# nyashiki/nshogi-engine

Hardware: NVIDIA B200
Metric: nn_leaf_evals_per_sec_batch256 (higher is better)
Workload: dtype bf16

## Files before the change

### nshogi-engine_b200/binding.py

```python
from __future__ import annotations

import ctypes as C
import os
from typing import Optional

import numpy as np

HERE = os.path.dirname(os.path.abspath(__file__))
LIB_PATH = os.path.join(HERE, "libnsb.so")

NUM_SQUARES = 81
POLICY_SIZE = 2187
FEATURE_CHANNELS = 86
MAX_LEGAL_MOVES = 593
CACHE_MAX_MOVES = 164
DECODE_PROBS = 0
DECODE_LOGITS = 1
DECODE_BOTH = 2
DECODE_NAN_FALLBACK = 0x100
ROW_SKIP_SOFTMAX = 1

FEATURE_BITBOARD = np.dtype([("lo", "<u8"), ("hi", "<u8")])
POSITION = np.dtype(
    {
# ... 255 lines not shown


class Event:

    def __init__(self):
        p = _P()
        _check(lib().nsb_event_create(C.byref(p)), "nsb_event_create")
        self._p = p

    def record(self, ctx: "Context", slot: int = 0):
        _check(ctx._l.nsb_event_record(self._p, ctx._h, slot), "nsb_event_record")

    def sync(self):
        _check(lib().nsb_event_sync(self._p), "nsb_event_sync")

    def elapsed_ms(self, stop: "Event") -> float:
        ms = C.c_float(0)
        _check(lib().nsb_event_elapsed_ms(self._p, stop._p, C.byref(ms)), "nsb_event_elapsed_ms")
        return float(ms.value)

    def destroy(self):
        if self._p is not None:
            lib().nsb_event_destroy(self._p)
            self._p = None


class Context:

    def __init__(self, desc: NetDesc, batch_max: int, slots: int = 1, gpu: int = 0,
                 blob: Optional[np.ndarray] = None, seed: Optional[int] = None, diag: bool = False):
        self.desc = desc
        self.batch_max = batch_max
        self.slots = slots
        self._l = diag_lib() if diag else lib()
        h = _P()
        _check(self._l.nsb_create(C.byref(h), gpu, batch_max, slots, C.byref(desc)), "nsb_create")
        self._h = h
        if blob is None and seed is not None:
            blob = random_blob(desc, seed)
        if blob is not None:
            self.load_weights(blob)

    def close(self):
        if self._h is not None:
            self._l.nsb_destroy(self._h)
            self._h = None

    def __enter__(self):
        return self

    def __exit__(self, *a):
        self.close()

    def load_weights(self, blob: np.ndarray):
        blob = np.ascontiguousarray(blob, dtype=np.float32)
        _check(self._l.nsb_load_weights(self._h, blob.ctypes.data, blob.size), "nsb_load_weights")

    def bind_thread(self):
        _check(self._l.nsb_bind_thread(self._h), "nsb_bind_thread")

    def eval_async(self, slot, features, n, policy, win, draw):
        _check(self._l.nsb_eval_async(self._h, slot, _ptr(features), n, _ptr(policy), _ptr(win), _ptr(draw)),
               "nsb_eval_async")

    def eval_decode_async(self, slot, features, n, move_off, move_idx, mode, legal_out, win, draw, nan_flag=None):
        _check(self._l.nsb_eval_decode_async(self._h, slot, _ptr(features), n, _ptr(move_off), _ptr(move_idx), mode,
                                           _ptr(legal_out), _ptr(win), _ptr(draw), _ptr(nan_flag)),
               "nsb_eval_decode_async")

    def eval_positions_async(self, slot, positions, n, policy, win, draw):
        _check(self._l.nsb_eval_positions_async(self._h, slot, _ptr(positions), n, _ptr(policy), _ptr(win),
                                              _ptr(draw)), "nsb_eval_positions_async")

    def eval_positions_decode_async(self, slot, positions, n, move_off, move_idx, mode, legal_out, win, draw,
                                    nan_flag=None):
        _check(self._l.nsb_eval_positions_decode_async(self._h, slot, _ptr(positions), n, _ptr(move_off),
                                                     _ptr(move_idx), mode, _ptr(legal_out), _ptr(win), _ptr(draw),
                                                     _ptr(nan_flag)), "nsb_eval_positions_decode_async")

    def await_(self, slot=0):
        _check(self._l.nsb_await(self._h, slot), "nsb_await")

    def is_computing(self, slot=0) -> bool:
        rc = self._l.nsb_is_computing(self._h, slot)
        if rc < 0:
            _check(rc, "nsb_is_computing")
        return rc == 1

    def eval_device(self, slot, d_features, n, d_policy, d_win, d_draw):
        _check(self._l.nsb_eval_device(self._h, slot, _ptr(d_features), n, _ptr(d_policy), _ptr(d_win), _ptr(d_draw)),
               "nsb_eval_device")

    def eval_decode_device(self, slot, d_features, n, d_off, d_idx, mode, d_policy, d_legal, d_win, d_draw, d_flag):
        _check(self._l.nsb_eval_decode_device(self._h, slot, _ptr(d_features), n, _ptr(d_off), _ptr(d_idx), mode,
                                            _ptr(d_policy), _ptr(d_legal), _ptr(d_win), _ptr(d_draw), _ptr(d_flag)),
               "nsb_eval_decode_device")

    def extract_device(self, slot, d_features, n, channels, channels_first, d_planes):
        _check(self._l.nsb_extract_device(self._h, slot, _ptr(d_features), n, channels, int(channels_first),
                                        _ptr(d_planes)), "nsb_extract_device")

    def pack_positions_device(self, slot, d_positions, n, d_features):
        _check(self._l.nsb_pack_positions_device(self._h, slot, _ptr(d_positions), n, _ptr(d_features)),
               "nsb_pack_positions_device")

    def decode_device(self, slot, d_policy, d_win, d_draw, n, d_off, d_idx, mode, d_legal, d_flag):
        _check(self._l.nsb_decode_device(self._h, slot, _ptr(d_policy), _ptr(d_win), _ptr(d_draw), n, _ptr(d_off),
                                       _ptr(d_idx), mode, _ptr(d_legal), _ptr(d_flag)), "nsb_decode_device")

    def decode_device_ex(self, slot, d_policy, d_win, d_draw, n, d_off, d_idx, mode, d_row_flags, d_legal, d_logits, d_flag):
        _check(self._l.nsb_decode_device_ex(self._h, slot, _ptr(d_policy), _ptr(d_win), _ptr(d_draw), n, _ptr(d_off),
                                          _ptr(d_idx), mode, _ptr(d_row_flags), _ptr(d_legal), _ptr(d_logits), _ptr(d_flag)),
               "nsb_decode_device_ex")

    def cache_create(self, memory_mb: int):
        _check(self._l.nsb_cache_create(self._h, memory_mb), "nsb_cache_create")

    def cache_clear(self):
        _check(self._l.nsb_cache_clear(self._h), "nsb_cache_clear")

    def cache_num_bundles(self) -> int:
        return int(self._l.nsb_cache_num_bundles(self._h))

    def cache_store_device(self, slot, d_hashes, n, d_off, d_legal, d_win, d_draw, d_skip=None, d_stored=None):
        _check(self._l.nsb_cache_store_device(self._h, slot, _ptr(d_hashes), n, _ptr(d_off), _ptr(d_legal), _ptr(d_win),
                                            _ptr(d_draw), _ptr(d_skip), _ptr(d_stored)), "nsb_cache_store_device")

    def cache_probe_device(self, slot, d_hashes, n, d_off, d_legal, d_win, d_draw, d_hit, d_miss_idx, d_miss_count):
        _check(self._l.nsb_cache_probe_device(self._h, slot, _ptr(d_hashes), n, _ptr(d_off), _ptr(d_legal), _ptr(d_win),
                                            _ptr(d_draw), _ptr(d_hit), _ptr(d_miss_idx), _ptr(d_miss_count)),
               "nsb_cache_probe_device")

    def eval_cached_decode_async(self, slot, features, n, hashes, move_off, move_idx, mode, legal_out, win, draw,
                                 nan_flag=None, hit_flag=None):
        _check(self._l.nsb_eval_cached_decode_async(self._h, slot, _ptr(features), n, _ptr(hashes), _ptr(move_off),
                                                  _ptr(move_idx), mode, _ptr(legal_out), _ptr(win), _ptr(draw),
                                                  _ptr(nan_flag), _ptr(hit_flag)), "nsb_eval_cached_decode_async")

    def eval_positions_cached_decode_async(self, slot, positions, n, hashes, move_off, move_idx, mode, legal_out, win,
                                           draw, nan_flag=None, hit_flag=None):
        _check(self._l.nsb_eval_positions_cached_decode_async(self._h, slot, _ptr(positions), n, _ptr(hashes),
                                                            _ptr(move_off), _ptr(move_idx), mode, _ptr(legal_out),
                                                            _ptr(win), _ptr(draw), _ptr(nan_flag), _ptr(hit_flag)),
               "nsb_eval_positions_cached_decode_async")

    def eval_cached_decode_device(self, slot, d_features, n, d_hashes, d_off, d_idx, mode, d_legal, d_win, d_draw,
                                  d_flag, d_hit):
        _check(self._l.nsb_eval_cached_decode_device(self._h, slot, _ptr(d_features), n, _ptr(d_hashes), _ptr(d_off),
                                                   _ptr(d_idx), mode, _ptr(d_legal), _ptr(d_win), _ptr(d_draw),
                                                   _ptr(d_flag), _ptr(d_hit)), "nsb_eval_cached_decode_device")

    def debug_trunk_timeline(self, slot, d_features, n, positions=False):
        nl = 2 * self.desc.blocks + 2
        out = np.zeros(nl * 4 + 16 + 3 * 1024, dtype=np.uint64)
        fn = self._l.nsb_debug_trunk_timeline_positions if positions else self._l.nsb_debug_trunk_timeline
        _check(fn(self._h, slot, _ptr(d_features), n, out.ctypes.data, out.size), "nsb_debug_trunk_timeline")
        return out[:nl * 4].reshape(nl, 4), out[nl * 4:]

    def eval_request_async(self, slot, n, move_off, move_idx, mode, legal_out, win, draw, features=None, positions=None,
                           hashes=None, order_out=None, nan_flag=None, hit_flag=None, row_flags=None, logits_out=None):
        r = DecodeRequest(_ptr(features), _ptr(positions), n, _ptr(hashes), _ptr(move_off), _ptr(move_idx), mode,
                          _ptr(legal_out), _ptr(order_out), _ptr(win), _ptr(draw), _ptr(nan_flag), _ptr(hit_flag),
                          _ptr(row_flags), _ptr(logits_out))
        _check(self._l.nsb_eval_request_async(self._h, slot, C.byref(r)), "nsb_eval_request_async")

    def cache_attach(self, owner: "Context"):
        _check(self._l.nsb_cache_attach(self._h, owner._h), "nsb_cache_attach")

    def set_io_mode(self, direct: bool):
        _check(self._l.nsb_set_io_mode(self._h, 1 if direct else 0), "nsb_set_io_mode")

    def io_mode(self) -> str:
        return "direct" if self._l.nsb_io_mode(self._h) == 1 else "staged"

    def stream(self, slot=0) -> int:
        return self._l.nsb_stream(self._h, slot) or 0

    def set_timing(self, on: bool):
        _check(self._l.nsb_set_timing(self._h, int(on)), "nsb_set_timing")

    def trunk_time(self):
        s, n = C.c_double(0), C.c_uint64(0)
        _check(self._l.nsb_trunk_time(self._h, C.byref(s), C.byref(n)), "nsb_trunk_time")
        return float(s.value), int(n.value)

    def trunk_time_reset(self):
        _check(self._l.nsb_trunk_time_reset(self._h), "nsb_trunk_time_reset")

    def trunk_kernel_name(self) -> str:
        return self._l.nsb_trunk_kernel_name(self._h).decode()

    def launch_count(self) -> int:
        return int(self._l.nsb_launch_count(self._h))
```

### nshogi-engine_b200/csrc/epilogue.cuh

```cuda
#pragma once
#include <stdint.h>

#include "umma.cuh"

namespace nsb {

__host__ __device__ constexpr bool is_real_slot(int n) { return (n % 100) < 90 && ((n % 100) % 10) < 9; }

template <int NCG>
struct EpilogueMask {
    uint32_t m[NCG * 4];
    template <int COL0>
    __device__ __forceinline__ void init_at(int lane) {
#pragma unroll
        for (int G = 0; G < NCG * 4; ++G) {
            uint32_t v = 0;
#pragma unroll
            for (int q4 = 0; q4 < 4; ++q4) {
                const int n = COL0 + 8 * G + 2 * q4;
                const uint32_t c = (is_real_slot(n) ? 0x0000FFFFu : 0u) | (is_real_slot(n + 1) ? 0xFFFF0000u : 0u);
                v = (lane & 3) == q4 ? c : v;
            }
            m[G] = v;
        }
    }
    __device__ __forceinline__ void init(int col0, int lane) {
        if (col0 == 0) init_at<0>(lane);
        else init_at<96>(lane);
    }
};

template <int NCG, bool kResidual, int LBS = 2>
__device__ __forceinline__ void epilogue_half(int lb, uint32_t taddr, uint32_t buf, uint32_t pitch, int chunk0,
                                              int col0, const float (&bias)[4], const EpilogueMask<NCG>& mask,
                                              int lane) {
    const int mk = lane >> 3, mi = lane & 7;
    uint32_t v[NCG][16];
#pragma unroll
    for (int cg = 0; cg < NCG; ++cg) tmem_ld_16x256b_x4(taddr + ((uint32_t)(lb * 16) << 16) + cg * 32, v[cg]);
    const uint32_t row_addr =
        buf + (uint32_t)(chunk0 + lb * LBS + (mk & 1)) * pitch + (uint32_t)(col0 + 8 * (mk >> 1) + mi) * 16u;
    uint32_t xr[NCG][2][4];
    if (kResidual) {
#pragma unroll
        for (int cg = 0; cg < NCG; ++cg)
#pragma unroll
            for (int h = 0; h < 2; ++h)
                ldmatrix_x4_trans(row_addr + (uint32_t)(cg * 32 + h * 16) * 16u, xr[cg][h][0], xr[cg][h][1],
                                  xr[cg][h][2], xr[cg][h][3]);
    }
    tmem_ld_wait();
    const float b0 = lb ? bias[2] : bias[0], b1 = lb ? bias[3] : bias[1];
    const uint64_t bb0 = pack_f32x2(b0, b0), bb1 = pack_f32x2(b1, b1);
#pragma unroll
    for (int cg = 0; cg < NCG; ++cg)
#pragma unroll
        for (int h = 0; h < 2; ++h) {
            uint32_t p[4];
#pragma unroll
            for (int m = 0; m < 4; ++m) {
                const int g = 2 * h + (m >> 1), rh = m & 1;
                uint64_t x = add_f32x2(pack_u32x2(v[cg][4 * g + 2 * rh + 0], v[cg][4 * g + 2 * rh + 1]), rh ? bb1 : bb0);
                if (kResidual) x = add_f32x2(x, pack_u32x2(xr[cg][h][m] << 16, xr[cg][h][m] & 0xFFFF0000u));
                p[m] = pack_relu_bf16x2(x) & mask.m[cg * 4 + g];
            }
            stmatrix_x4_trans(row_addr + (uint32_t)(cg * 32 + h * 16) * 16u, p[0], p[1], p[2], p[3]);
        }
}

template <int NCG, bool kResidual>
__device__ __forceinline__ void epilogue_warp(uint32_t taddr, uint32_t buf, uint32_t pitch, int chunk0, int col0,
                                              const float (&bias)[4], const EpilogueMask<NCG>& mask, int lane) {
#pragma unroll
    for (int lb = 0; lb < 2; ++lb)
        epilogue_half<NCG, kResidual>(lb, taddr, buf, pitch, chunk0, col0, bias, mask, lane);
}

}
```

### nshogi-engine_b200/csrc/nsb_api.cu

```cuda
#include <cuda_runtime.h>
#include <stdarg.h>
#include <stdio.h>
#include <stdlib.h>
#include <string.h>

#include <map>
#include <mutex>
#include <new>
#include <vector>

#include "nsb_internal.h"
#ifdef NSB_DIAG
#include "../../include/nsb_diag.h"
#endif

namespace nsb {

static thread_local char g_err[512] = "";

void set_error(const char* fmt, ...) {
    va_list ap;
    va_start(ap, fmt);
    vsnprintf(g_err, sizeof g_err, fmt, ap);
    va_end(ap);
// ... 863 lines not shown
    r.features = features;
    r.n = n;
    r.hashes = hashes;
    r.move_off = move_off;
    r.move_idx = move_idx;
    r.mode = mode;
    r.legal_out = legal_out;
    r.win = win;
    r.draw = draw;
    r.nan_flag = nan_flag;
    r.hit_flag = hit_flag;
    int rc = check_cache(c, slot, "nsb_eval_cached_decode_async");
    if (rc) return rc;
    if (!features || !hashes) {
        set_error("nsb_eval_cached_decode_async: null buffer or bad mode");
        return NSB_ERR_INVALID;
    }
    return eval_request(c, slot, r, "nsb_eval_cached_decode_async");
}

int nsb_eval_positions_cached_decode_async(nsb_ctx* c, int slot, const nsb_position* positions, size_t n,
                                           const uint64_t* hashes, const uint32_t* move_off, const uint16_t* move_idx,
                                           int mode, float* legal_out, float* win, float* draw, uint8_t* nan_flag,
                                           uint8_t* hit_flag) {
    nsb_decode_request r{};
    r.positions = positions;
    r.n = n;
    r.hashes = hashes;
    r.move_off = move_off;
    r.move_idx = move_idx;
    r.mode = mode;
    r.legal_out = legal_out;
    r.win = win;
    r.draw = draw;
    r.nan_flag = nan_flag;
    r.hit_flag = hit_flag;
    int rc = check_cache(c, slot, "nsb_eval_positions_cached_decode_async");
    if (rc) return rc;
    if (!positions || !hashes) {
        set_error("nsb_eval_positions_cached_decode_async: null buffer or bad mode");
        return NSB_ERR_INVALID;
    }
    return eval_request(c, slot, r, "nsb_eval_positions_cached_decode_async");
}

static int eval_request(nsb_ctx* c, int slot, const nsb_decode_request& r, const char* who) {
    int rc = r.hashes ? check_cache(c, slot, who) : check_ctx(c, slot);
    if (rc) return rc;
    const size_t n = r.n;
    if ((rc = check_batch(c, n, true))) return rc;
    if ((r.features != nullptr) == (r.positions != nullptr) || !r.move_off || !r.move_idx || !r.legal_out || !r.win || !r.draw ||
        !mode_ok(r.mode)) {
        set_error("%s: null buffer or bad mode", who);
        return NSB_ERR_INVALID;
    }
    if (r.positions && (rc = check_positions_net(c, who))) return rc;
    if (n == 0) return 0;
    if ((rc = check_offsets(r.move_off, n, who))) return rc;
    const size_t total = r.move_off[n];
    const bool both = (r.mode & NSB_DECODE_MODE_MASK) == NSB_DECODE_BOTH;
    const uint8_t* row_flags = both ? r.row_flags : nullptr;
    float* logits_out = both ? r.logits_out : nullptr;
    Slot& s = c->slots[slot];
    const size_t in_bytes = r.features ? n * (size_t)c->desc.in_channels * sizeof(nsb_feature_bitboard) : n * sizeof(nsb_position);
    const void* in = r.features ? (const void*)r.features : (const void*)r.positions;

    EvalArgs a{};
    a.n = (int)n;
    a.decode_mode = r.mode;
    const bool direct = c->direct_io && (r.features || c->fuse_pack) && host_mapped(in, in_bytes) &&
                        decode_buffers_mapped(n, total, r.move_off, r.move_idx, r.legal_out, r.win, r.draw, r.nan_flag) &&
                        (!r.hashes || host_mapped(r.hashes, n * sizeof(uint64_t))) && (!r.hit_flag || host_mapped(r.hit_flag, n)) &&
                        (!r.order_out || host_mapped(r.order_out, (total ? total : 1) * sizeof(uint16_t))) &&
                        (!row_flags || host_mapped(row_flags, n)) &&
                        (!logits_out || host_mapped(logits_out, (total ? total : 1) * sizeof(float)));
    const uint64_t* hashes = r.hashes;
    uint8_t* hit = r.hit_flag ? r.hit_flag : s.d_hit;
    if (direct) {
        a.features = r.features;
        a.positions = r.positions;
        a.win = r.win;
        a.draw = r.draw;
        a.move_off = r.move_off;
        a.move_idx = r.move_idx;
        a.legal_out = r.legal_out;
        a.order_out = r.order_out;
        a.nan_flag = r.nan_flag ? r.nan_flag : (r.hashes ? s.d_flag : nullptr);
        a.row_flags = row_flags;
        a.logits_out = logits_out;
    } else {
        NSB_CUDA(cudaMemcpyAsync(r.features ? (void*)s.d_feat : (void*)s.d_pos, in, in_bytes, cudaMemcpyHostToDevice, s.stream));
        a.features = s.d_feat;
        if (r.positions && (rc = stage1(c, s, n, &a.positions))) return rc;
        if (r.hashes) {
            NSB_CUDA(cudaMemcpyAsync(s.d_hash, r.hashes, n * sizeof(uint64_t), cudaMemcpyHostToDevice, s.stream));
            hashes = s.d_hash;
            hit = s.d_hit;
        }
        NSB_CUDA(cudaMemcpyAsync(s.d_off, r.move_off, (n + 1) * sizeof(uint32_t), cudaMemcpyHostToDevice, s.stream));
        if (total)
            NSB_CUDA(cudaMemcpyAsync(s.d_idx, r.move_idx, total * sizeof(uint16_t), cudaMemcpyHostToDevice, s.stream));
        a.win = s.d_win;
        a.draw = s.d_draw;
        a.move_off = s.d_off;
        a.move_idx = s.d_idx;
        a.legal_out = s.d_legal;
        a.order_out = r.order_out ? s.d_order : nullptr;
        a.nan_flag = s.d_flag;
        if (row_flags) {
            NSB_CUDA(cudaMemcpyAsync(s.d_rowflags, row_flags, n, cudaMemcpyHostToDevice, s.stream));
            a.row_flags = s.d_rowflags;
        }
        if (logits_out) {
            if (!s.d_logits) NSB_CUDA(cudaMalloc(&s.d_logits, (size_t)c->batch_max * NSB_MAX_LEGAL_MOVES * sizeof(float)));
            a.logits_out = s.d_logits;
        }
    }
    if (r.hashes) {
        NSB_CUDA(cudaMemsetAsync(s.d_miss_count, 0, sizeof(int), s.stream));
        int k = launch_cache_probe(c->cache, hashes, n, a.move_off, a.legal_out, a.win, a.draw, hit, a.nan_flag, s.d_miss_idx,
                                   s.d_miss_count, s.stream, a.order_out, r.mode, a.row_flags, a.logits_out);
        NSB_CUDA(cudaGetLastError());
        c->launches += (uint64_t)k;
        a.index = s.d_miss_idx;
        a.count = s.d_miss_count;
        a.hashes = hashes;
        a.cache = c->cache;
    }
    if ((rc = run_trunk(c, s, a))) return rc;
    if (direct) return 0;
    if (total) {
        NSB_CUDA(cudaMemcpyAsync(r.legal_out, s.d_legal, total * sizeof(float), cudaMemcpyDeviceToHost, s.stream));
        if (r.order_out)
            NSB_CUDA(cudaMemcpyAsync(r.order_out, s.d_order, total * sizeof(uint16_t), cudaMemcpyDeviceToHost, s.stream));
        if (logits_out)
            NSB_CUDA(cudaMemcpyAsync(logits_out, s.d_logits, total * sizeof(float), cudaMemcpyDeviceToHost, s.stream));
    }
    NSB_CUDA(cudaMemcpyAsync(r.win, s.d_win, n * sizeof(float), cudaMemcpyDeviceToHost, s.stream));
    NSB_CUDA(cudaMemcpyAsync(r.draw, s.d_draw, n * sizeof(float), cudaMemcpyDeviceToHost, s.stream));
    if (r.nan_flag) NSB_CUDA(cudaMemcpyAsync(r.nan_flag, s.d_flag, n, cudaMemcpyDeviceToHost, s.stream));
    if (r.hashes && r.hit_flag) NSB_CUDA(cudaMemcpyAsync(r.hit_flag, s.d_hit, n, cudaMemcpyDeviceToHost, s.stream));
    return 0;
}

#ifdef NSB_DIAG
static int debug_timeline(nsb_ctx* c, int slot, const nsb_feature_bitboard* d_features, const nsb_position* d_positions,
                          size_t n, uint64_t* host_stamps, size_t max_stamps) {
    int rc = check_ctx(c, slot);
    if (rc) return rc;
    if (!c->loaded || (!d_features && !d_positions) || !host_stamps || n == 0) {
        set_error("nsb_debug_trunk_timeline: bad arguments or weights not loaded");
        return NSB_ERR_INVALID;
    }
    const size_t need = (size_t)c->net.num_layers * 4 + 16 + 3 * 1024;
    if (max_stamps < need) {
        set_error("nsb_debug_trunk_timeline: need room for %zu stamps", need);
        return NSB_ERR_INVALID;
    }
    Slot& s = c->slots[slot];
    unsigned long long* d_t = nullptr;
    NSB_CUDA(cudaMalloc(&d_t, need * 8));
    NSB_CUDA(cudaMemsetAsync(d_t, 0, need * 8, s.stream));
    EvalArgs a{};
    a.features = d_features;
    a.positions = d_positions;
    a.n = (int)n;
    a.policy = s.d_policy;
    a.win = s.d_win;
    a.draw = s.d_draw;
    a.timeline = d_t;
    if (n > (size_t)c->batch_max) {
        cudaFree(d_t);
        set_error("nsb_debug_trunk_timeline: n exceeds batch_max");
        return NSB_ERR_INVALID;
    }
    rc = run_trunk(c, s, a);
    if (rc == 0) {
        cudaError_t e = cudaStreamSynchronize(s.stream);
        if (e == cudaSuccess) e = cudaMemcpy(host_stamps, d_t, need * 8, cudaMemcpyDeviceToHost);
        if (e != cudaSuccess) {
            set_error("nsb_debug_trunk_timeline: %s", cudaGetErrorString(e));
            rc = NSB_ERR_CUDA;
        }
    }
    cudaFree(d_t);
    return rc;
}

int nsb_debug_trunk_timeline(nsb_ctx* c, int slot, const nsb_feature_bitboard* d_features, size_t n,
                             uint64_t* host_stamps, size_t max_stamps) {
    return debug_timeline(c, slot, d_features, nullptr, n, host_stamps, max_stamps);
}

int nsb_debug_trunk_timeline_positions(nsb_ctx* c, int slot, const nsb_position* d_positions, size_t n,
                                       uint64_t* host_stamps, size_t max_stamps) {
    return debug_timeline(c, slot, nullptr, d_positions, n, host_stamps, max_stamps);
}

#endif

int nsb_extract_device(nsb_ctx* c, int slot, const nsb_feature_bitboard* d_features, size_t n, int channels,
                       int channels_first, float* d_planes) {
    int rc = check_ctx(c, slot);
    if (rc) return rc;
    if (!d_features || !d_planes || channels < 1 || channels > 1024) {
        set_error("nsb_extract_device: bad arguments");
        return NSB_ERR_INVALID;
    }
    int k = launch_extract(d_features, n, channels, channels_first, d_planes, c->slots[slot].stream);
    if (k < 0) return k;
    NSB_CUDA(cudaGetLastError());
    c->launches += (uint64_t)k;
    return 0;
}

int nsb_pack_positions_device(nsb_ctx* c, int slot, const nsb_position* d_positions, size_t n,
                              nsb_feature_bitboard* d_features) {
    int rc = check_ctx(c, slot);
    if (rc) return rc;
    if (!d_positions || !d_features) {
        set_error("nsb_pack_positions_device: null buffer");
        return NSB_ERR_INVALID;
    }
    int k = launch_pack_positions(d_positions, n, d_features, c->slots[slot].stream);
    if (k < 0) return k;
    NSB_CUDA(cudaGetLastError());
    c->launches += (uint64_t)k;
    return 0;
}

int nsb_decode_device(nsb_ctx* c, int slot, const float* d_policy, const float* d_win, const float* d_draw,
                      size_t n, const uint32_t* d_move_off, const uint16_t* d_move_idx, int mode,
                      float* d_legal_out, uint8_t* d_nan_flag) {
    int rc = check_ctx(c, slot);
    if (rc) return rc;
    return nsb_decode_device_ex(c, slot, d_policy, d_win, d_draw, n, d_move_off, d_move_idx, mode, nullptr, d_legal_out,
                                nullptr, d_nan_flag);
}

int nsb_decode_device_ex(nsb_ctx* c, int slot, const float* d_policy, const float* d_win, const float* d_draw,
                         size_t n, const uint32_t* d_move_off, const uint16_t* d_move_idx, int mode,
                         const uint8_t* d_row_flags, float* d_legal_out, float* d_logits_out, uint8_t* d_nan_flag) {
    int rc = check_ctx(c, slot);
    if (rc) return rc;
    if (!d_policy || !d_win || !d_draw || !d_move_off || !d_move_idx || !d_legal_out || !mode_ok(mode)) {
        set_error("nsb_decode_device: null buffer or bad mode");
        return NSB_ERR_INVALID;
    }
    int k = launch_decode(d_policy, d_win, d_draw, n, d_move_off, d_move_idx, mode, d_legal_out, d_nan_flag,
                          c->slots[slot].stream, d_row_flags, d_logits_out);
    if (k < 0) return k;
    NSB_CUDA(cudaGetLastError());
    c->launches += (uint64_t)k;
    return 0;
}

void* nsb_stream(nsb_ctx* c, int slot) {
    if (check_ctx(c, slot)) return nullptr;
    return c->slots[slot].stream;
}

int nsb_set_timing(nsb_ctx* c, int enabled) {
    if (!c) {
        set_error("null ctx");
        return NSB_ERR_INVALID;
    }
    c->timing = enabled != 0;
    return 0;
}

int nsb_trunk_time(nsb_ctx* c, double* sum_ms, uint64_t* launches) {
    if (!c) {
        set_error("null ctx");
        return NSB_ERR_INVALID;
    }
    if (sum_ms) *sum_ms = c->trunk_ms;
    if (launches) *launches = c->trunk_launches;
    return 0;
}

int nsb_trunk_time_reset(nsb_ctx* c) {
    if (!c) {
        set_error("null ctx");
        return NSB_ERR_INVALID;
    }
    c->trunk_ms = 0.0;
    c->trunk_launches = 0;
    return 0;
}

uint64_t nsb_launch_count(nsb_ctx* c) { return c ? c->launches : 0; }


int nsb_host_alloc(void** out, size_t bytes) {
    if (!out) return NSB_ERR_INVALID;
    NSB_CUDA(cudaHostAlloc(out, bytes ? bytes : 1, cudaHostAllocPortable | cudaHostAllocMapped));
    std::lock_guard<std::mutex> lock(g_host_mu);
    g_host_allocs[(uintptr_t)*out] = HostRange{bytes ? bytes : 1, true, HostKind::Alloc};
    return 0;
}
int nsb_host_alloc_near(void** out, size_t bytes, int gpu) {
    if (!out) return NSB_ERR_INVALID;
    int node = -1;
    void* p = alloc_near_gpu(bytes ? bytes : 1, gpu, &node);
    if (!p) {
        set_error("nsb_host_alloc_near: mmap of %zu bytes failed", bytes);
        return NSB_ERR_NOMEM;
// ... 173 lines not shown
```

### nshogi-engine_b200/csrc/trunk_tmem.cu

```cuda
#include <cuda_bf16.h>
#include <cuda_runtime.h>
#include <stdint.h>

#include "trunk_common.cuh"

namespace nsb {

namespace {

template <int NGRP_>
struct TmemGeom {
    static constexpr int C = 128;
    static constexpr int KCH = C / 8;
    static constexpr int NGRP = NGRP_;
    static constexpr int NPOS = 2;
    static constexpr int QPOS = NGRP * NPOS;
    static constexpr int NCOLS = NPOS * 96;
    static constexpr int GUARD = 12;
    static constexpr int SPITCH = (GUARD + NCOLS + 11) | 1;
    static constexpr int BUF_BYTES = ((KCH * SPITCH * 16 + 127) / 128) * 128;
    static constexpr int KC64 = C / 64;
    static constexpr int TMEM_COLS = 256 * NGRP;
    static constexpr int A_COL0 = NGRP * NCOLS;
    static constexpr int A_STAGES = 4 * NGRP;
    static constexpr int A_STAGE_COLS = 16;
    static constexpr int THREADS = 128 * (2 + NGRP);
    static constexpr int GRP_THREADS = 128;
    static constexpr int EPI_WARPS = GRP_THREADS / 32;
    static constexpr int MMA_WARP = 4 + 4 * NGRP;
    static constexpr int MIN_BLOCKS = NGRP == 1 ? 2 : 1;
    static constexpr int PRODUCER_REGS = 72, EPI_REGS = NGRP == 1 ? 128 : 168, MMA_REGS = 40;
    static constexpr int NBARS = 2 * A_STAGES + 2;
    static constexpr int SCRATCH_BYTES = ((NPOS * kPolicySize * 4 + 15) / 16) * 16;
    static constexpr int FEAT_BYTES = NPOS * kMaxInChannels * 16;
    static constexpr int VBUF_BYTES = ((NPOS * 81 * 4 + 15) / 16) * 16;
    static constexpr int RED_BYTES = ((EPI_WARPS * NPOS * 2 * 4 + NPOS * 2 * 4 + 15) / 16) * 16;
    static constexpr int GRP_BYTES = 2 * BUF_BYTES;
    static constexpr int OFF_BUF_A = 0;
    static constexpr int OFF_BUF_B = BUF_BYTES;
    static constexpr int OFF_VBUF = NGRP * GRP_BYTES;
    static constexpr int OFF_RED = OFF_VBUF + NGRP * VBUF_BYTES;
    static constexpr int OFF_BARS = OFF_RED + NGRP * RED_BYTES;
    static constexpr int SMEM_BYTES = OFF_BARS + NBARS * 8 + 16 + 128;
    static_assert(BUF_BYTES == 55040, "each group has the duo kernel's activation layout");
    static_assert(NGRP > 1 || (OFF_VBUF == 110080 && OFF_RED == 110736 && OFF_BARS == 110816 && SMEM_BYTES == 111040),
                  "one group keeps the duo kernel's shared memory map");
    static_assert(SCRATCH_BYTES <= BUF_BYTES && FEAT_BYTES <= BUF_BYTES, "aliases fit into buffer A");
    static_assert(A_COL0 + A_STAGES * A_STAGE_COLS == TMEM_COLS, "accumulators + the ring fill the allocation");
    static_assert(MIN_BLOCKS * (SMEM_BYTES + 1024) <= 233472, "MIN_BLOCKS CTAs per SM");
    static_assert(128 * (PRODUCER_REGS + NGRP * EPI_REGS + MMA_REGS) <= 65536 / MIN_BLOCKS,
                  "re-balanced registers of MIN_BLOCKS CTAs fit the SM");
};

template <int NGRP>
__device__ __forceinline__ void trunk_tmem_body(const DeviceNet& net, const EvalArgs& a) {
    using G = TmemGeom<NGRP>;
    constexpr int C = G::C;
    extern __shared__ uint8_t smem_raw[];
    uint8_t* smem = reinterpret_cast<uint8_t*>(((uintptr_t)smem_raw + 127) & ~(uintptr_t)127);
    const uint32_t sbase = smem_u32(smem);
    const uint32_t bars = sbase + G::OFF_BARS;
    auto bar_afull = [&](int s) { return bars + 8u * s; };
    auto bar_aempty = [&](int s) { return bars + 8u * (G::A_STAGES + s); };
    const uint32_t bar_act = bars + 8u * (2 * G::A_STAGES);
    const uint32_t bar_acc = bars + 8u * (2 * G::A_STAGES + 1);
    volatile uint32_t* tmem_holder = reinterpret_cast<volatile uint32_t*>(smem + G::OFF_BARS + 8 * G::NBARS);

    const int warp = threadIdx.x >> 5, lane = threadIdx.x & 31;
    const int n_eff = eval_count(a);
    const int units = (n_eff + G::QPOS - 1) / G::QPOS;
    const int my_passes =
        (int)blockIdx.x < units ? (units - (int)blockIdx.x + (int)gridDim.x - 1) / (int)gridDim.x : 0;
    const int NL = net.num_layers;
    const bool stamp = eval_timeline(a) && blockIdx.x == 0;
    unsigned long long* cta_rec = (eval_timeline(a) && blockIdx.x < 1024) ? eval_timeline(a) + 4 * NL + 16 + 3 * blockIdx.x : nullptr;
    if (cta_rec && threadIdx.x == 0) {
        unsigned smid;
        unsigned long long t;
        asm volatile("mov.u32 %0, %%smid;" : "=r"(smid));
        asm volatile("mov.u64 %0, %%globaltimer;" : "=l"(t));
        cta_rec[0] = smid;
        cta_rec[1] = t;
    }

    for (int i = threadIdx.x; i < G::NGRP * G::GRP_BYTES / 16; i += G::THREADS)
        reinterpret_cast<uint4*>(smem)[i] = make_uint4(0, 0, 0, 0);
    if (threadIdx.x == 0) {
        for (int s = 0; s < G::A_STAGES; ++s) {
            mbar_init(bar_afull(s), 4);
            mbar_init(bar_aempty(s), 1);
        }
        mbar_init(bar_act, G::NGRP * G::EPI_WARPS);
        mbar_init(bar_acc, 1);
        fence_mbar_init();
    }
    fence_proxy_async_smem();
    if (warp == G::MMA_WARP) tmem_alloc(smem_u32(const_cast<uint32_t*>(tmem_holder)), G::TMEM_COLS);
    tc_fence_before();
    __syncthreads();
    tc_fence_after();
    const uint32_t tmem_base = *tmem_holder;

    if (warp < 4) {
        setmaxnreg_dec<G::PRODUCER_REGS>();
        const int row = threadIdx.x;
        const uint32_t lane_addr = tmem_base + ((uint32_t)(warp * 32) << 16) + G::A_COL0;
        const int steps_per_pass = net.stages_per_pass;
        uint32_t slot = 0, phase = 0;
        auto load_stage = [&](uint4 (&dst)[4], const uint4* s) {
            dst[0] = __ldg(s);
            dst[1] = __ldg(s + 1);
            dst[2] = __ldg(s + 256);
            dst[3] = __ldg(s + 257);
        };
        auto store_stage = [&](const uint4 (&buf)[4]) {
            mbar_wait(bar_aempty(slot), phase ^ 1u);
            tc_fence_after();
            asm volatile(
                "tcgen05.st.sync.aligned.32x32b.x16.b32 [%0], "
                "{%1, %2, %3, %4, %5, %6, %7, %8, %9, %10, %11, %12, %13, %14, %15, %16};"
                ::"r"(lane_addr + slot * G::A_STAGE_COLS), "r"(buf[0].x), "r"(buf[0].y), "r"(buf[0].z), "r"(buf[0].w),
                  "r"(buf[1].x), "r"(buf[1].y), "r"(buf[1].z), "r"(buf[1].w), "r"(buf[2].x), "r"(buf[2].y), "r"(buf[2].z),
                  "r"(buf[2].w), "r"(buf[3].x), "r"(buf[3].y), "r"(buf[3].z), "r"(buf[3].w)
                : "memory");
            tmem_st_wait();
            tc_fence_before();
            __syncwarp();
            if (lane == 0) mbar_arrive(bar_afull(slot));
            if (++slot == G::A_STAGES) { slot = 0; phase ^= 1u; }
        };
        const int stages_per_pass = steps_per_pass / 2;
        for (int p = 0; p < my_passes; ++p) {
            const uint4* src = reinterpret_cast<const uint4*>(net.tiles) + (size_t)row * 2;
            uint4 b0[4], b1[4], b2[4];
            int ld = 0, st = 0;
            if (ld < stages_per_pass) { load_stage(b0, src + (size_t)ld * 512); ++ld; }
            if (ld < stages_per_pass) { load_stage(b1, src + (size_t)ld * 512); ++ld; }
            if (ld < stages_per_pass) { load_stage(b2, src + (size_t)ld * 512); ++ld; }
            for (;;) {
                store_stage(b0); ++st;
                if (ld < stages_per_pass) { load_stage(b0, src + (size_t)ld * 512); ++ld; }
                if (st >= stages_per_pass) break;
                store_stage(b1); ++st;
                if (ld < stages_per_pass) { load_stage(b1, src + (size_t)ld * 512); ++ld; }
                if (st >= stages_per_pass) break;
                store_stage(b2); ++st;
                if (ld < stages_per_pass) { load_stage(b2, src + (size_t)ld * 512); ++ld; }
                if (st >= stages_per_pass) break;
            }
        }
    } else if (warp >= G::MMA_WARP) {
        setmaxnreg_dec<G::MMA_REGS>();
        if (warp == G::MMA_WARP) {
            constexpr uint32_t idesc = make_idesc_bf16_f32(128, G::NCOLS);
            constexpr uint32_t b_lbo = G::SPITCH * 16;
            uint32_t slot = 0, phase = 0, act_phase = 0;
            for (int p = 0; p < my_passes; ++p) {
                for (int L = 0; L < NL; ++L) {
                    mbar_wait(bar_act, act_phase);
                    act_phase ^= 1u;
                    tc_fence_after();
                    if (stamp && p == 0 && lane == 0) eval_timeline(a)[4 * L + 0] = clock64();
                    const bool head = (L == NL - 1);
                    const uint32_t in_buf = sbase + ((L & 1) ? G::OFF_BUF_A : G::OFF_BUF_B);
                    const int ntaps = head ? 1 : 9;
                    for (int kc = 0; kc < G::KC64; ++kc) {
                        const int halves = block_steps(net, L, kc) / 2;
                        for (int tap = 0; tap < ntaps; ++tap) {
                            const int shift = head ? 0 : (tap / 3 - 1) * 10 + (tap % 3 - 1);
                            const uint32_t b_base = in_buf + (uint32_t)((kc * 8 * G::SPITCH + G::GUARD + shift) * 16);
                            if (halves == 2) {
                                const uint32_t s0 = slot, s1 = (slot + 1) % G::A_STAGES;
                                const uint32_t ph1 = s1 == 0 ? phase ^ 1u : phase;
                                mbar_wait(bar_afull(s0), phase);
                                mbar_wait(bar_afull(s1), ph1);
                                tc_fence_after();
                                if (elect_one()) {
#pragma unroll
                                    for (int h = 0; h < 2; ++h) {
                                        const uint32_t a_base = tmem_base + G::A_COL0 + (h ? s1 : s0) * G::A_STAGE_COLS;
#pragma unroll
                                        for (int g = 0; g < G::NGRP; ++g) {
                                            const uint32_t b_lo = smem_desc_lo(b_base + g * G::GRP_BYTES, b_lbo);
#pragma unroll
                                            for (int k2 = 0; k2 < 2; ++k2) {
                                                const int k = 2 * h + k2;
                                                umma_bf16_ts(tmem_base + g * G::NCOLS, a_base + k2 * 8,
                                                             smem_desc_from(b_lo + (uint32_t)(2 * k * G::SPITCH), 128),
                                                             idesc, (uint32_t)((kc | tap | k) != 0));
                                            }
                                        }
                                        umma_commit(bar_aempty(h ? s1 : s0));
                                    }
                                }
                                __syncwarp();
                                slot = (slot + 2) % G::A_STAGES;
                                if (slot < 2) phase ^= 1u;
                                continue;
                            }
                            for (int h = 0; h < halves; ++h) {
                                mbar_wait(bar_afull(slot), phase);
                                tc_fence_after();
                                if (elect_one()) {
                                    const uint32_t a_base = tmem_base + G::A_COL0 + slot * G::A_STAGE_COLS;
#pragma unroll
                                    for (int g = 0; g < G::NGRP; ++g) {
                                        const uint32_t b_lo =
                                            smem_desc_lo(b_base + g * G::GRP_BYTES, b_lbo) + (uint32_t)(4 * h * G::SPITCH);
#pragma unroll
                                        for (int k2 = 0; k2 < 2; ++k2)
                                            umma_bf16_ts(tmem_base + g * G::NCOLS, a_base + k2 * 8,
                                                         smem_desc_from(b_lo + (uint32_t)(2 * k2 * G::SPITCH), 128),
                                                         idesc, (uint32_t)((kc | tap | h | k2) != 0));
                                    }
                                    umma_commit(bar_aempty(slot));
                                }
                                __syncwarp();
                                if (++slot == G::A_STAGES) { slot = 0; phase ^= 1u; }
                            }
                        }
                    }
                    if (elect_one()) umma_commit(bar_acc);
                    __syncwarp();
                    if (stamp && p == 0 && lane == 0) eval_timeline(a)[4 * L + 1] = clock64();
                }
            }
        }
    } else {
        setmaxnreg_inc<G::EPI_REGS>();
        const int g = NGRP == 1 ? 0 : (warp - 4) >> 2;
        const int et = threadIdx.x - 128 - g * G::GRP_THREADS;
        const int q = warp & 3;
        const uint32_t bar = kEpiBar + g;
        uint8_t* gsmem = smem + g * G::GRP_BYTES;
        const uint32_t bufA = sbase + g * G::GRP_BYTES + G::OFF_BUF_A, bufB = sbase + g * G::GRP_BYTES + G::OFF_BUF_B;
        float* scratch = reinterpret_cast<float*>(gsmem + G::OFF_BUF_A);
        uint4* featS = reinterpret_cast<uint4*>(gsmem + G::OFF_BUF_A);
        float* vbuf = reinterpret_cast<float*>(smem + G::OFF_VBUF + g * G::VBUF_BYTES);
        float* red = reinterpret_cast<float*>(smem + G::OFF_RED + g * G::RED_BYTES);
        const uint32_t taddr = tmem_base + ((uint32_t)(q * 32) << 16) + g * G::NCOLS;
        const bool stamper = stamp && g == 0 && et == 0;
        EpilogueMask<3> mask0, mask1;
        mask0.init(0, lane);
        mask1.init(96, lane);
        uint32_t acc_phase = 0;
        for (int p = 0; p < my_passes; ++p) {
            const int b0 = ((int)blockIdx.x + p * (int)gridDim.x) * G::QPOS + g * G::NPOS;

            expand_features<G::NPOS, G::SPITCH, G::GUARD, G::GRP_THREADS>(net, a, n_eff, b0, featS, gsmem + G::OFF_BUF_B, et, nullptr, bar);
            named_bar_sync(bar, G::GRP_THREADS);
            for (int i = et; i < G::FEAT_BYTES / 16; i += G::GRP_THREADS) featS[i] = make_uint4(0, 0, 0, 0);
            fence_proxy_async_smem();
            __syncwarp();
            if (lane == 0) mbar_arrive(bar_act);

            for (int L = 0; L < NL - 1; ++L) {
                float bias[4];
#pragma unroll
                for (int k = 0; k < 4; ++k)
                    bias[k] = __ldg(net.bias + (size_t)L * C + 64 * (k >> 1) + 16 * q + 8 * (k & 1) + (lane >> 2));
                mbar_wait(bar_acc, acc_phase);
                acc_phase ^= 1u;
                tc_fence_after();
                if (stamper && p == 0) eval_timeline(a)[4 * L + 2] = clock64();
                const uint32_t out_buf = ((L & 1) ? bufB : bufA) + G::GUARD * 16;
                const bool residual = (L >= 2) && ((L & 1) == 0);
#pragma unroll
                for (int part = 0; part < 2; ++part)
#pragma unroll
                    for (int lb = 0; lb < 2; ++lb) {
                        if (residual)
                            epilogue_half<3, true, 8>(lb, taddr + 96 * part, out_buf, G::SPITCH * 16, 2 * q, 96 * part, bias,
                                                      part ? mask1 : mask0, lane);
                        else
                            epilogue_half<3, false, 8>(lb, taddr + 96 * part, out_buf, G::SPITCH * 16, 2 * q, 96 * part, bias,
                                                       part ? mask1 : mask0, lane);
                    }
                tc_fence_before();
                fence_proxy_async_smem();
                __syncwarp();
                if (lane == 0) mbar_arrive(bar_act);
                if (stamper && p == 0) eval_timeline(a)[4 * L + 3] = clock64();
            }

            const int hp = 7 * q + lane;
            const float hbias = lane < 7 ? __ldg(net.bias + (size_t)(NL - 1) * C + hp) : 0.f;
            mbar_wait(bar_acc, acc_phase);
            acc_phase ^= 1u;
            tc_fence_after();
            head_read<0>(taddr, hbias, hp, scratch, vbuf, lane);
            head_read<96>(taddr + 96, hbias, hp, scratch, vbuf, lane);
            tc_fence_before();
            named_bar_sync(bar, G::GRP_THREADS);
            heads_tail_small<G::NPOS, G::GRP_THREADS>(net, a, n_eff, b0, scratch, vbuf, red, et, bar);
            if (p + 1 < my_passes) {
                for (int i = et; i < G::SCRATCH_BYTES / 16; i += G::GRP_THREADS)
                    reinterpret_cast<uint4*>(scratch)[i] = make_uint4(0, 0, 0, 0);
                named_bar_sync(bar, G::GRP_THREADS);
            }
        }
    }

    tc_fence_before();
    __syncthreads();
    if (cta_rec && threadIdx.x == 0) {
        unsigned long long t;
        asm volatile("mov.u64 %0, %%globaltimer;" : "=l"(t));
        cta_rec[2] = t;
    }
    if (warp == G::MMA_WARP) {
        __syncwarp();
        tmem_dealloc(tmem_base, G::TMEM_COLS);
    }
}

__global__ void __launch_bounds__(TmemGeom<1>::THREADS, TmemGeom<1>::MIN_BLOCKS)
    trunk_duo_kernel(const DeviceNet net, const EvalArgs a) { trunk_tmem_body<1>(net, a); }
__global__ void __launch_bounds__(TmemGeom<2>::THREADS, TmemGeom<2>::MIN_BLOCKS)
    trunk_quad_kernel(const DeviceNet net, const EvalArgs a) { trunk_tmem_body<2>(net, a); }

template <int NGRP>
constexpr auto tmem_kernel = NGRP == 1 ? trunk_duo_kernel : trunk_quad_kernel;

template <int NGRP>
int tmem_prepare(int* ctas_per_sm) {
    using G = TmemGeom<NGRP>;
    cudaError_t e = cudaFuncSetAttribute(tmem_kernel<NGRP>, cudaFuncAttributeMaxDynamicSharedMemorySize, G::SMEM_BYTES);
    if (e == cudaSuccess)
        e = cudaFuncSetAttribute(tmem_kernel<NGRP>, cudaFuncAttributePreferredSharedMemoryCarveout, 100);
    int nb = 0;
    if (e == cudaSuccess)
        e = cudaOccupancyMaxActiveBlocksPerMultiprocessor(&nb, tmem_kernel<NGRP>, G::THREADS, G::SMEM_BYTES);
    if (e != cudaSuccess || nb < 1) {
        set_error("trunk %s: cannot configure the kernel: %s (is this an sm_100a device?)", NGRP == 1 ? "duo" : "quad",
                  cudaGetErrorString(e));
        return NSB_ERR_NO_DEVICE;
    }
    if (ctas_per_sm) *ctas_per_sm = nb < G::MIN_BLOCKS ? G::MIN_BLOCKS : nb;
    return 0;
}

template <int NGRP>
int tmem_launch(const DeviceNet& net, const EvalArgs& a, int num_sms, int ctas_per_sm, cudaStream_t s) {
    using G = TmemGeom<NGRP>;
    if (a.n <= 0) return 0;
    const int units = (a.n + G::QPOS - 1) / G::QPOS;
    const int cap = num_sms * (ctas_per_sm > 0 ? ctas_per_sm : 1);
    const int grid = units < cap ? units : cap;
    tmem_kernel<NGRP><<<grid, G::THREADS, G::SMEM_BYTES, s>>>(net, a);
    return 1;
}

}

int trunk_duo_prepare(int* ctas_per_sm) { return tmem_prepare<1>(ctas_per_sm); }

int launch_trunk_duo(const DeviceNet& net, const EvalArgs& a, int num_sms, int ctas_per_sm, cudaStream_t s) {
    return tmem_launch<1>(net, a, num_sms, ctas_per_sm, s);
}

int trunk_quad_prepare() { return tmem_prepare<2>(nullptr); }

int launch_trunk_quad(const DeviceNet& net, const EvalArgs& a, int num_sms, cudaStream_t s) {
    return tmem_launch<2>(net, a, num_sms, 1, s);
}

}
```

Measured before the change: 2.600 million.

## Split epilogue into two halves with separate barrier so next-layer MMA starts early

For multi-group configurations the epilogue now writes the first K-chunk half (lb=0) of the activation buffer and signals the MMA warp via the existing barrier, then stores the held lb=1 results and signals a new second mbarrier. The MMA warp waits on that second barrier only before its second K chunk, so next-layer MMAs can overlap the epilogue's remaining stores. Residual skip loads are also issued before waiting on the accumulator. This raises epilogue register budget to 200 to hold results, risking spills or lower occupancy, and adds timeline stamps for the new arrival point.

```diff
diff --git a/nshogi-engine_b200/binding.py b/nshogi-engine_b200/binding.py
--- a/nshogi-engine_b200/binding.py
+++ b/nshogi-engine_b200/binding.py
@@ -431,10 +431,11 @@
 
     def debug_trunk_timeline(self, slot, d_features, n, positions=False):
         nl = 2 * self.desc.blocks + 2
-        out = np.zeros(nl * 4 + 16 + 3 * 1024, dtype=np.uint64)
+        out = np.zeros(nl * 5 + 16 + 3 * 1024, dtype=np.uint64)
         fn = self._l.nsb_debug_trunk_timeline_positions if positions else self._l.nsb_debug_trunk_timeline
         _check(fn(self._h, slot, _ptr(d_features), n, out.ctypes.data, out.size), "nsb_debug_trunk_timeline")
-        return out[:nl * 4].reshape(nl, 4), out[nl * 4:]
+        rest = nl * 4 + 16 + 3 * 1024
+        return np.concatenate([out[:nl * 4].reshape(nl, 4), out[rest:, None]], axis=1), out[nl * 4:rest]
 
     def eval_request_async(self, slot, n, move_off, move_idx, mode, legal_out, win, draw, features=None, positions=None,
                            hashes=None, order_out=None, nan_flag=None, hit_flag=None, row_flags=None, logits_out=None):
diff --git a/nshogi-engine_b200/csrc/epilogue.cuh b/nshogi-engine_b200/csrc/epilogue.cuh
--- a/nshogi-engine_b200/csrc/epilogue.cuh
+++ b/nshogi-engine_b200/csrc/epilogue.cuh
@@ -30,25 +30,46 @@
     }
 };
 
+template <int LBS>
+__device__ __forceinline__ uint32_t epilogue_row_addr(int lb, uint32_t buf, uint32_t pitch, int chunk0, int col0,
+                                                      int lane) {
+    const int mk = lane >> 3, mi = lane & 7;
+    return buf + (uint32_t)(chunk0 + lb * LBS + (mk & 1)) * pitch + (uint32_t)(col0 + 8 * (mk >> 1) + mi) * 16u;
+}
+
+template <int NCG>
+__device__ __forceinline__ void epilogue_skip_load(uint32_t row_addr, uint32_t (&xr)[NCG][2][4]) {
+#pragma unroll
+    for (int cg = 0; cg < NCG; ++cg)
+#pragma unroll
+        for (int h = 0; h < 2; ++h)
+            ldmatrix_x4_trans(row_addr + (uint32_t)(cg * 32 + h * 16) * 16u, xr[cg][h][0], xr[cg][h][1], xr[cg][h][2],
+                              xr[cg][h][3]);
+}
+
+template <int NCG, bool kResidual>
+__device__ __forceinline__ void epilogue_pack(const uint32_t (&v)[16], const uint32_t (&xr)[4], int cg, int h,
+                                              uint64_t bb0, uint64_t bb1, const EpilogueMask<NCG>& mask,
+                                              uint32_t (&p)[4]) {
+#pragma unroll
+    for (int m = 0; m < 4; ++m) {
+        const int g = 2 * h + (m >> 1), rh = m & 1;
+        uint64_t x = add_f32x2(pack_u32x2(v[4 * g + 2 * rh + 0], v[4 * g + 2 * rh + 1]), rh ? bb1 : bb0);
+        if (kResidual) x = add_f32x2(x, pack_u32x2(xr[m] << 16, xr[m] & 0xFFFF0000u));
+        p[m] = pack_relu_bf16x2(x) & mask.m[cg * 4 + g];
+    }
+}
+
 template <int NCG, bool kResidual, int LBS = 2>
 __device__ __forceinline__ void epilogue_half(int lb, uint32_t taddr, uint32_t buf, uint32_t pitch, int chunk0,
                                               int col0, const float (&bias)[4], const EpilogueMask<NCG>& mask,
                                               int lane) {
-    const int mk = lane >> 3, mi = lane & 7;
     uint32_t v[NCG][16];
 #pragma unroll
     for (int cg = 0; cg < NCG; ++cg) tmem_ld_16x256b_x4(taddr + ((uint32_t)(lb * 16) << 16) + cg * 32, v[cg]);
-    const uint32_t row_addr =
-        buf + (uint32_t)(chunk0 + lb * LBS + (mk & 1)) * pitch + (uint32_t)(col0 + 8 * (mk >> 1) + mi) * 16u;
+    const uint32_t row_addr = epilogue_row_addr<LBS>(lb, buf, pitch, chunk0, col0, lane);
     uint32_t xr[NCG][2][4];
-    if (kResidual) {
-#pragma unroll
-        for (int cg = 0; cg < NCG; ++cg)
-#pragma unroll
-            for (int h = 0; h < 2; ++h)
-                ldmatrix_x4_trans(row_addr + (uint32_t)(cg * 32 + h * 16) * 16u, xr[cg][h][0], xr[cg][h][1],
-                                  xr[cg][h][2], xr[cg][h][3]);
-    }
+    if (kResidual) epilogue_skip_load<NCG>(row_addr, xr);
     tmem_ld_wait();
     const float b0 = lb ? bias[2] : bias[0], b1 = lb ? bias[3] : bias[1];
     const uint64_t bb0 = pack_f32x2(b0, b0), bb1 = pack_f32x2(b1, b1);
@@ -57,15 +78,35 @@
 #pragma unroll
         for (int h = 0; h < 2; ++h) {
             uint32_t p[4];
-#pragma unroll
-            for (int m = 0; m < 4; ++m) {
-                const int g = 2 * h + (m >> 1), rh = m & 1;
-                uint64_t x = add_f32x2(pack_u32x2(v[cg][4 * g + 2 * rh + 0], v[cg][4 * g + 2 * rh + 1]), rh ? bb1 : bb0);
-                if (kResidual) x = add_f32x2(x, pack_u32x2(xr[cg][h][m] << 16, xr[cg][h][m] & 0xFFFF0000u));
-                p[m] = pack_relu_bf16x2(x) & mask.m[cg * 4 + g];
-            }
+            epilogue_pack<NCG, kResidual>(v[cg], xr[cg][h], cg, h, bb0, bb1, mask, p);
             stmatrix_x4_trans(row_addr + (uint32_t)(cg * 32 + h * 16) * 16u, p[0], p[1], p[2], p[3]);
         }
+}
+
+template <int NCG, bool kResidual>
+__device__ __forceinline__ void epilogue_half_regs(int lb, uint32_t taddr, const float (&bias)[4],
+                                                   const EpilogueMask<NCG>& mask, const uint32_t (&xr)[NCG][2][4],
+                                                   uint32_t (&p)[NCG][2][4]) {
+    uint32_t v[NCG][16];
+#pragma unroll
+    for (int cg = 0; cg < NCG; ++cg) tmem_ld_16x256b_x4(taddr + ((uint32_t)(lb * 16) << 16) + cg * 32, v[cg]);
+    tmem_ld_wait();
+    const float b0 = lb ? bias[2] : bias[0], b1 = lb ? bias[3] : bias[1];
+    const uint64_t bb0 = pack_f32x2(b0, b0), bb1 = pack_f32x2(b1, b1);
+#pragma unroll
+    for (int cg = 0; cg < NCG; ++cg)
+#pragma unroll
+        for (int h = 0; h < 2; ++h) epilogue_pack<NCG, kResidual>(v[cg], xr[cg][h], cg, h, bb0, bb1, mask, p[cg][h]);
+}
+
+template <int NCG>
+__device__ __forceinline__ void epilogue_store(uint32_t row_addr, const uint32_t (&p)[NCG][2][4]) {
+#pragma unroll
+    for (int cg = 0; cg < NCG; ++cg)
+#pragma unroll
+        for (int h = 0; h < 2; ++h)
+            stmatrix_x4_trans(row_addr + (uint32_t)(cg * 32 + h * 16) * 16u, p[cg][h][0], p[cg][h][1], p[cg][h][2],
+                              p[cg][h][3]);
 }
 
 template <int NCG, bool kResidual>
diff --git a/nshogi-engine_b200/csrc/nsb_api.cu b/nshogi-engine_b200/csrc/nsb_api.cu
--- a/nshogi-engine_b200/csrc/nsb_api.cu
+++ b/nshogi-engine_b200/csrc/nsb_api.cu
@@ -1039,7 +1039,7 @@
         set_error("nsb_debug_trunk_timeline: bad arguments or weights not loaded");
         return NSB_ERR_INVALID;
     }
-    const size_t need = (size_t)c->net.num_layers * 4 + 16 + 3 * 1024;
+    const size_t need = (size_t)c->net.num_layers * 5 + 16 + 3 * 1024;
     if (max_stamps < need) {
         set_error("nsb_debug_trunk_timeline: need room for %zu stamps", need);
         return NSB_ERR_INVALID;
diff --git a/nshogi-engine_b200/csrc/trunk_tmem.cu b/nshogi-engine_b200/csrc/trunk_tmem.cu
--- a/nshogi-engine_b200/csrc/trunk_tmem.cu
+++ b/nshogi-engine_b200/csrc/trunk_tmem.cu
@@ -1,6 +1,8 @@
 #include <cuda_bf16.h>
 #include <cuda_runtime.h>
 #include <stdint.h>
+
+#include <type_traits>
 
 #include "trunk_common.cuh"
 
@@ -29,8 +31,8 @@
     static constexpr int EPI_WARPS = GRP_THREADS / 32;
     static constexpr int MMA_WARP = 4 + 4 * NGRP;
     static constexpr int MIN_BLOCKS = NGRP == 1 ? 2 : 1;
-    static constexpr int PRODUCER_REGS = 72, EPI_REGS = NGRP == 1 ? 128 : 168, MMA_REGS = 40;
-    static constexpr int NBARS = 2 * A_STAGES + 2;
+    static constexpr int PRODUCER_REGS = 72, EPI_REGS = NGRP == 1 ? 128 : 200, MMA_REGS = 40;
+    static constexpr int NBARS = 2 * A_STAGES + 2 + (NGRP > 1);
     static constexpr int SCRATCH_BYTES = ((NPOS * kPolicySize * 4 + 15) / 16) * 16;
     static constexpr int FEAT_BYTES = NPOS * kMaxInChannels * 16;
     static constexpr int VBUF_BYTES = ((NPOS * 81 * 4 + 15) / 16) * 16;
@@ -64,6 +66,7 @@
     auto bar_aempty = [&](int s) { return bars + 8u * (G::A_STAGES + s); };
     const uint32_t bar_act = bars + 8u * (2 * G::A_STAGES);
     const uint32_t bar_acc = bars + 8u * (2 * G::A_STAGES + 1);
+    const uint32_t bar_act1 = bars + 8u * (2 * G::A_STAGES + 2);
     volatile uint32_t* tmem_holder = reinterpret_cast<volatile uint32_t*>(smem + G::OFF_BARS + 8 * G::NBARS);
 
     const int warp = threadIdx.x >> 5, lane = threadIdx.x & 31;
@@ -92,6 +95,7 @@
         }
         mbar_init(bar_act, G::NGRP * G::EPI_WARPS);
         mbar_init(bar_acc, 1);
+        if (NGRP > 1) mbar_init(bar_act1, G::NGRP * G::EPI_WARPS);
         fence_mbar_init();
     }
     fence_proxy_async_smem();
@@ -154,7 +158,7 @@
         if (warp == G::MMA_WARP) {
             constexpr uint32_t idesc = make_idesc_bf16_f32(128, G::NCOLS);
             constexpr uint32_t b_lbo = G::SPITCH * 16;
-            uint32_t slot = 0, phase = 0, act_phase = 0;
+            uint32_t slot = 0, phase = 0, act_phase = 0, act1_phase = 0;
             for (int p = 0; p < my_passes; ++p) {
                 for (int L = 0; L < NL; ++L) {
                     mbar_wait(bar_act, act_phase);
@@ -165,6 +169,11 @@
                     const uint32_t in_buf = sbase + ((L & 1) ? G::OFF_BUF_A : G::OFF_BUF_B);
                     const int ntaps = head ? 1 : 9;
                     for (int kc = 0; kc < G::KC64; ++kc) {
+                        if (NGRP > 1 && kc == 1) {
+                            mbar_wait(bar_act1, act1_phase);
+                            act1_phase ^= 1u;
+                            tc_fence_after();
+                        }
                         const int halves = block_steps(net, L, kc) / 2;
                         for (int tap = 0; tap < ntaps; ++tap) {
                             const int shift = head ? 0 : (tap / 3 - 1) * 10 + (tap % 3 - 1);
@@ -252,35 +261,82 @@
             for (int i = et; i < G::FEAT_BYTES / 16; i += G::GRP_THREADS) featS[i] = make_uint4(0, 0, 0, 0);
             fence_proxy_async_smem();
             __syncwarp();
-            if (lane == 0) mbar_arrive(bar_act);
+            if (lane == 0) {
+                mbar_arrive(bar_act);
+                if (NGRP > 1) mbar_arrive(bar_act1);
+            }
 
             for (int L = 0; L < NL - 1; ++L) {
                 float bias[4];
 #pragma unroll
                 for (int k = 0; k < 4; ++k)
                     bias[k] = __ldg(net.bias + (size_t)L * C + 64 * (k >> 1) + 16 * q + 8 * (k & 1) + (lane >> 2));
-                mbar_wait(bar_acc, acc_phase);
-                acc_phase ^= 1u;
-                tc_fence_after();
-                if (stamper && p == 0) eval_timeline(a)[4 * L + 2] = clock64();
                 const uint32_t out_buf = ((L & 1) ? bufB : bufA) + G::GUARD * 16;
                 const bool residual = (L >= 2) && ((L & 1) == 0);
-#pragma unroll
-                for (int part = 0; part < 2; ++part)
-#pragma unroll
-                    for (int lb = 0; lb < 2; ++lb) {
-                        if (residual)
-                            epilogue_half<3, true, 8>(lb, taddr + 96 * part, out_buf, G::SPITCH * 16, 2 * q, 96 * part, bias,
-                                                      part ? mask1 : mask0, lane);
-                        else
-                            epilogue_half<3, false, 8>(lb, taddr + 96 * part, out_buf, G::SPITCH * 16, 2 * q, 96 * part, bias,
-                                                       part ? mask1 : mask0, lane);
-                    }
-                tc_fence_before();
-                fence_proxy_async_smem();
-                __syncwarp();
-                if (lane == 0) mbar_arrive(bar_act);
-                if (stamper && p == 0) eval_timeline(a)[4 * L + 3] = clock64();
+                if constexpr (NGRP == 1) {
+                    mbar_wait(bar_acc, acc_phase);
+                    acc_phase ^= 1u;
+                    tc_fence_after();
+                    if (stamper && p == 0) eval_timeline(a)[4 * L + 2] = clock64();
+#pragma unroll
+                    for (int part = 0; part < 2; ++part)
+#pragma unroll
+                        for (int lb = 0; lb < 2; ++lb) {
+                            if (residual)
+                                epilogue_half<3, true, 8>(lb, taddr + 96 * part, out_buf, G::SPITCH * 16, 2 * q, 96 * part,
+                                                          bias, part ? mask1 : mask0, lane);
+                            else
+                                epilogue_half<3, false, 8>(lb, taddr + 96 * part, out_buf, G::SPITCH * 16, 2 * q, 96 * part,
+                                                           bias, part ? mask1 : mask0, lane);
+                        }
+                    tc_fence_before();
+                    fence_proxy_async_smem();
+                    __syncwarp();
+                    if (lane == 0) mbar_arrive(bar_act);
+                    if (stamper && p == 0) eval_timeline(a)[4 * L + 3] = clock64();
+                } else {
+                    auto row = [&](int lb, int part) {
+                        return epilogue_row_addr<8>(lb, out_buf, G::SPITCH * 16, 2 * q, 96 * part, lane);
+                    };
+                    auto split_epilogue = [&](auto residual_t) {
+                        constexpr bool kRes = decltype(residual_t)::value;
+                        uint32_t xr[2][2][3][2][4];
+                        if (kRes) {
+                            epilogue_skip_load<3>(row(1, 0), xr[0][1]);
+                            epilogue_skip_load<3>(row(1, 1), xr[1][1]);
+                            epilogue_skip_load<3>(row(0, 0), xr[0][0]);
+                        }
+                        mbar_wait(bar_acc, acc_phase);
+                        acc_phase ^= 1u;
+                        tc_fence_after();
+                        if (stamper && p == 0) eval_timeline(a)[4 * L + 2] = clock64();
+                        uint32_t held[2][3][2][4];
+#pragma unroll
+                        for (int part = 0; part < 2; ++part)
+                            epilogue_half_regs<3, kRes>(1, taddr + 96 * part, bias, part ? mask1 : mask0, xr[part][1],
+                                                        held[part]);
+                        if (kRes) epilogue_skip_load<3>(row(0, 1), xr[1][0]);
+#pragma unroll
+                        for (int part = 0; part < 2; ++part) {
+                            uint32_t p0[3][2][4];
+                            epilogue_half_regs<3, kRes>(0, taddr + 96 * part, bias, part ? mask1 : mask0, xr[part][0], p0);
+                            epilogue_store<3>(row(0, part), p0);
+                        }
+                        tc_fence_before();
+                        fence_proxy_async_smem();
+                        __syncwarp();
+                        if (lane == 0) mbar_arrive(bar_act);
+                        if (stamper && p == 0) eval_timeline(a)[4 * L + 3] = clock64();
+#pragma unroll
+                        for (int part = 0; part < 2; ++part) epilogue_store<3>(row(1, part), held[part]);
+                        fence_proxy_async_smem();
+                        __syncwarp();
+                        if (lane == 0) mbar_arrive(bar_act1);
+                        if (stamper && p == 0) eval_timeline(a)[4 * NL + 16 + 3 * 1024 + L] = clock64();
+                    };
+                    if (residual) split_epilogue(std::true_type{});
+                    else split_epilogue(std::false_type{});
+                }
             }
 
             const int hp = 7 * q + lane;
```

Result: faster. 2.631 million, median of 6 (+1.2%).
